# pagmerek/frave

Measured on AMD Instinct MI355X. Metric: Mpixels/s encode (transform+quant) at 4096x4096, higher is better.
Workload: dtype u8->i32

## Files before the change

frave_amd/csrc/fri_hip.cpp:

```cpp
#include "fri_hip_internal.hpp"

#include <atomic>
#include <cstdio>
#include <cstdlib>
#include <mutex>
#include <new>
#include <optional>
#include <thread>

#include "search_scaffold.hpp"
#include "solve6.hpp"

using namespace fri;
using namespace fri::host;

void PlanDelete::operator()(fri_hip_plan *p) const { delete p; }

struct fri_hip_multi {
    std::vector<fri_hip_ctx *> ctxs;
    std::vector<fri_hip_plan *> plans;
};

namespace {

// ... 12 lines not shown
std::vector<float> laplace_table() {
    static const float width[10] = {2.5f, 4.5f, 6.3f, 8.5f, 12.7f, 16.f, 20.f, 24.f, 28.f, 36.f};
    std::vector<float> t(10 * 1024);
    for (int b = 0; b < 10; b++)
        for (uint32_t j = 0; j < 1024; j++) {
            const float x = (float)((j & 1u) ? (int32_t)(j + 1) / -2 : (int32_t)(j / 2));
            t[b * 1024 + j] = std::exp(-std::fabs(x - 0.0f) / width[b]) / (2.0f * width[b]);
        }
    return t;
}

struct Knobs {
    int band_rows = 0, cells_per_tile = 0, cells_per_wg = 0, target_wgs = 0, tile_bytes = 0;
    int ranks = 0;
    std::optional<int> strided_shares;
    bool has_rank_weights = false;
    float rank_weight[4] = {0, 0, 0, 0};
    bool pins_forward = false;
    int batch_share_tiles = 0;
    std::optional<int> inv_shared, inv_strided_shares;
    int inv_band_rows = 0;
    int pred_blocks = 0, hist_blocks = 0, trace = 0, k3_scan = 0;
    int k1_ablate = 0, k2_ablate = 0, k3_ablate = 0, k4_ablate = 0;
    std::optional<int> k1_cached_stores, k1_batch_shares, k4_older_eighths;
};

Knobs read_knobs() {
    Knobs k;
    const char *on = std::getenv("FRI_HIP_TUNING");
    if (!on || on[0] != '1' || on[1] != 0) return k;
    auto env = [](const char *name) { return std::getenv(name); };
    auto pin = [&](const char *name) {
        const char *s = env(name);
        k.pins_forward |= s != nullptr;
        return s;
    };
    auto opt = [](const char *s) { return s ? std::optional<int>(std::atoi(s)) : std::nullopt; };
    auto num = [&](const char *s) { return opt(s).value_or(0); };
    k.band_rows = num(pin("FRI_HIP_BAND_ROWS")), k.cells_per_tile = num(pin("FRI_HIP_CELLS_PER_TILE")), k.cells_per_wg = num(pin("FRI_HIP_CELLS_PER_WG"));
    k.target_wgs = num(pin("FRI_HIP_TARGET_WGS")), k.tile_bytes = num(pin("FRI_HIP_TILE_BYTES")), k.ranks = std::min(num(pin("FRI_HIP_RANKS")), 4);
    k.strided_shares = opt(pin("FRI_HIP_STRIDED_SHARES"));
    if (const char *s = pin("FRI_HIP_RANK_WEIGHTS")) {
        float *w = k.rank_weight;
        k.has_rank_weights = std::sscanf(s, "%f,%f,%f,%f", &w[0], &w[1], &w[2], &w[3]) == 4;
    }
    k.batch_share_tiles = num(env("FRI_HIP_BATCH_SHARE_TILES"));
    k.inv_shared = opt(env("FRI_HIP_INV_SHARED")), k.inv_strided_shares = opt(env("FRI_HIP_INV_STRIDED_SHARES")), k.inv_band_rows = num(env("FRI_HIP_INV_BAND_ROWS"));
    k.pred_blocks = num(env("FRI_HIP_PRED_BLOCKS")), k.hist_blocks = num(env("FRI_HIP_HIST_BLOCKS")), k.trace = num(env("FRI_HIP_TRACE")), k.k3_scan = num(env("FRI_HIP_K3_SCAN"));
    k.k1_ablate = num(env("FRI_HIP_K1_ABLATE")), k.k2_ablate = num(env("FRI_HIP_K2_ABLATE")), k.k3_ablate = num(env("FRI_HIP_K3_ABLATE")), k.k4_ablate = num(env("FRI_HIP_K4_ABLATE"));
    k.k1_cached_stores = opt(env("FRI_HIP_K1_CACHED_STORES")), k.k1_batch_shares = opt(env("FRI_HIP_K1_BATCH_SHARES")), k.k4_older_eighths = opt(env("FRI_HIP_K4_OLDER_EIGHTHS"));
    return k;
}

int acquire_acc(fri_hip_plan *p, hipStream_t stream, uint32_t n_planes = 1) {
    fri_hip_ctx *c = p->ctx;
    HIP_TRY(c, hipSetDevice(c->device));
    if (p->acc_dirty) {
        HIP_TRY(c, hipDeviceSynchronize());
        for (auto &a : p->acc_slots) {
            if (a.pred_acc) HIP_TRY(c, hipMemset(a.pred_acc, 0, (size_t)a.planes * kPredAccWords * sizeof(uint32_t)));
            if (a.fit_acc) HIP_TRY(c, hipMemset(a.fit_acc, 0, (size_t)a.planes * kFitShards * kFitAccWords * sizeof(unsigned long long)));
        }
        HIP_TRY(c, hipDeviceSynchronize());
        p->acc_dirty = false;
    }
    int idx = -1;
    for (uint32_t i = 0; i < kPredAccRing && idx < 0; i++)
        if (p->acc_slots[i].used && p->acc_slots[i].stream == stream) idx = (int)i;
    for (uint32_t i = 0; i < kPredAccRing && idx < 0; i++)
        if (!p->acc_slots[i].used) {
            p->acc_slots[i].used = true;
            p->acc_slots[i].stream = stream;
            idx = (int)i;
// ... 480 lines not shown
            (e = upload(bufs, gi.inv_parts, d.inv_parts, kInvListPad)))
            return fail_hip(ctx, e, "inverse lists");
        d.inv_rect_bytes = gi.inv_rect_bytes;
    }
    d.F = (uint32_t)g.centers.size(), d.width = (int32_t)g.width, d.height = (int32_t)g.height, d.channels = (int32_t)g.channels, d.n_pred_tiles = g.n_pred_tiles;
    d.covers_image = g.n_valid_leaves == (uint64_t)g.width * g.height;
    d.inv_group = fwd.many_shares && g.wg_tiles.size() > 1 && (g.wg_tiles.size() - 1) % 1024 == 0 ? (int32_t)((g.wg_tiles.size() - 1) / 1024) : 1;
    d.inv_max_wg_tiles = d.inv_group > 1 ? 0 : d.max_wg_tiles, d.inv_max_wg_cells = d.inv_group > 1 ? 0 : d.max_wg_cells;
    for (size_t sh = 0; d.inv_group > 1 && sh + d.inv_group < g.wg_tiles.size(); sh += d.inv_group) {
        const Tile &first = g.tiles[g.wg_tiles[sh]], &last = g.tiles[g.wg_tiles[sh + d.inv_group] - 1];
        d.inv_max_wg_cells = std::max(d.inv_max_wg_cells, last.cell_begin + last.cell_count - first.cell_begin);
        d.inv_max_wg_tiles = std::max(d.inv_max_wg_tiles, g.wg_tiles[sh + d.inv_group] - g.wg_tiles[sh]);
    }
    d.pred_blocks = k.pred_blocks > 0 ? (uint32_t)k.pred_blocks : (uint32_t)ctx->cu_count;
    d.hist_blocks = k.hist_blocks > 0 ? (uint32_t)k.hist_blocks : 2u * (uint32_t)ctx->cu_count;
    d.k1_ablate = k.k1_ablate;
    if (k.k1_cached_stores) d.k1_cached_stores = *k.k1_cached_stores > 0 ? 1 : 0;
    if (k.k1_batch_shares) d.k1_batch_shares = *k.k1_batch_shares != 0;
    d.k2_ablate = k.k2_ablate;
    d.k3_ablate = k.k3_ablate;
    d.k3_scan = k.k3_scan > 0;
    d.k4_ablate = k.k4_ablate;
    if (k.k4_older_eighths) d.k4_older_eighths = *k.k4_older_eighths;
    if (hipMalloc(bufs.emplace_back().put(), (size_t)d.pred_blocks * kPredJunkWaves * kPredJunkBytes) != hipSuccess) return FRI_HIP_ERR_HIP;
    d.junk = static_cast<uint8_t *>(bufs.back().get());
    if (k.trace > 0) {
        const size_t bytes = (size_t)std::max<size_t>(d.n_wg, p->own_inverse_tiling ? gi.wg_tiles.size() : 0) * 16 * sizeof(unsigned long long);
        auto &t = bufs.emplace_back();
        if (hipMalloc(t.put(), bytes) != hipSuccess || hipMemset(t, 0, bytes) != hipSuccess) return FRI_HIP_ERR_HIP;
        d.trace = static_cast<unsigned long long *>(t.get());
    }
    if (hipEventCreate(p->ev_begin.put()) != hipSuccess || hipEventCreate(p->ev_end.put()) != hipSuccess) return FRI_HIP_ERR_HIP;
    p->dev_inv = d;
    if (p->own_inverse_tiling && (e = upload_tiling(bufs, gi, p->dev_inv, true))) return fail_hip(ctx, e, "inverse tiling");
    p->fwd_tunable = p->own_inverse_tiling && !fwd.many_shares && !d.trace && !k.pins_forward;
    if (p->fwd_tunable) adopt_cached_forward_tiling(p);
    *out = plan.release();
    return FRI_HIP_OK;
}

int fri_hip_plan_destroy(fri_hip_plan *p) {
    if (p && p->ctx) (void)hipSetDevice(p->ctx->device);
    delete p;
    return FRI_HIP_OK;
}

// ... 543 lines not shown
    const bool direct = d_node_words == nullptr;
    if (direct && !compact) return FRI_HIP_ERR_INVALID_ARGUMENT;
    if (compact) coef_stride = image;
    if (direct) word_stride = image;
    if (n_images > 1 && (pixel_stride < fri_hip_plan_pixel_bytes(p) || coef_stride < image || word_stride < image || symbol_stride < (size_t)C * n)) return FRI_HIP_ERR_INVALID_ARGUMENT;
    if (C > 1 && n_images > 1 && (coef_stride != image || word_stride != image || symbol_stride != (size_t)C * n)) return FRI_HIP_ERR_INVALID_ARGUMENT;
    QMatrix q;
    if (int rc = check_q(qmatrix, q)) return rc;
    hipStream_t s = (hipStream_t)stream;
    if (int rc = refuse_capture(p, s)) return rc;
    HIP_TRY(p->ctx, hipSetDevice(p->ctx->device));
    std::optional<Coefs16Lease> lease;
    if (compact && lease.emplace(p, s, (size_t)n_images * C).rc) return lease->rc;
    HIP_TRY(p->ctx, launch_fwd_transform_quant(p->dev, n_images, d_pixels, pixel_stride, d_coefs, coef_stride, q, s, chain_wants_cached_coefficients(p, n_images, fit),
                                               compact ? p->coefs16.get() : nullptr));
    PredBatch b;
    b.n_planes = n_images * C;
    b.coefs = d_coefs;
    b.coefs16 = compact ? p->coefs16.get() : nullptr;
    b.coef_stride = C > 1 || compact ? plane : coef_stride;
    b.out_stride = C > 1 ? plane : word_stride;
    b.params = reinterpret_cast<const PredictParams *>(d_params);
    b.words = d_node_words;
    if (direct) b.words = d_symbols, b.out_stride = C > 1 ? n : symbol_stride, b.stream_pos = p->d_stream_pos;
    if (fit)
        if (int rc = fit_chain(p, b, (unsigned long long *)d_fit_out_of_range, s, nullptr, nullptr, kPredForwardOutput)) return rc;
    if (int rc = predict_launch(p, b, nullptr, nullptr, d_hist, d_n_out_of_alphabet, kPredForwardOutput, s)) return rc;
    if (!direct) HIP_TRY(p->ctx, launch_symbol_gather(p->d_stream_order, n, b.n_planes, d_node_words, b.out_stride, d_symbols, C > 1 ? n : symbol_stride, s));
    return FRI_HIP_OK;
}

int fri_hip_fit_value_params_batch_dev(fri_hip_plan *p, uint32_t n_planes, const int64_t *d_gram, float *d_params, void *stream) {
    if (int rc = need_device(p)) return rc;
    if (!d_gram || !d_params || !n_planes || n_planes > 65535u) return FRI_HIP_ERR_INVALID_ARGUMENT;
    HIP_TRY(p->ctx, hipSetDevice(p->ctx->device));
    HIP_TRY(p->ctx, launch_fit_solve(0, n_planes, reinterpret_cast<const unsigned long long *>(d_gram), nullptr, nullptr, d_params, (hipStream_t)stream));
    return FRI_HIP_OK;
}

int fri_hip_fit_width_params_batch_dev(fri_hip_plan *p, uint32_t n_planes, const int64_t *d_wtw, const double *d_wtr, float *d_params, void *stream) {
    if (int rc = need_device(p)) return rc;
    if (!d_wtw || !d_wtr || !d_params || !n_planes || n_planes > 65535u) return FRI_HIP_ERR_INVALID_ARGUMENT;
    HIP_TRY(p->ctx, hipSetDevice(p->ctx->device));
    const uint64_t F = p->geo.centers.size();
    const unsigned long long rows[3] = {F * 256, F * 128, F * 128};
    HIP_TRY(p->ctx, launch_fit_solve(1, n_planes, reinterpret_cast<const unsigned long long *>(d_wtw), d_wtr, rows, d_params, (hipStream_t)stream));
    return FRI_HIP_OK;
}

int fri_hip_fit_params_batch_dev(fri_hip_plan *p, uint32_t n_planes, const int32_t *d_coefs, size_t coef_stride, float *d_params, uint64_t *d_fit_out_of_range, void *stream) {
    if (int rc = need_device(p)) return rc;
// ... 557 lines not shown
```

frave_amd/csrc/k2_predict.hip:

```cpp
#include "gather_common.hpp"

#include <algorithm>
#include <vector>

namespace fri {
namespace {

__device__ __forceinline__ uint32_t f32_as_u32(float x) {
    uint32_t r;
    asm("v_cvt_u32_f32 %0, %1" : "=v"(r) : "v"(x));
    return r;
}
__device__ __forceinline__ int f32_as_i32(float x) {
    int r;
    asm("v_cvt_i32_f32 %0, %1" : "=v"(r) : "v"(x));
    return r;
}
__host__ __device__ constexpr uint32_t bucket_of(uint32_t w) {
    return w < 3 ? 0 : w < 5 ? 1 : w < 6 ? 2 : w < 8 ? 3 : w < 12 ? 4 : w < 16 ? 5 : w < 20 ? 6 : w < 25 ? 7 : w < 30 ? 8 : 9;
}
__host__ __device__ constexpr uint32_t bucket_plane(int bit) {
    uint32_t m = 0;
    for (uint32_t w = 0; w < 32; w++) m |= ((bucket_of(w) >> bit) & 1u) << w;
    return m;
// ... 14 lines not shown
    const uint16_t *nbr_table;
    const uint32_t *pred_off;
    const uint16_t *pair_pos;
    const uint16_t *heap_of_pos;
    const uint32_t *halo_list;
    uint32_t *inexact;
    size_t coef_stride, out_stride;
    const PredictParams *params;
    int32_t ablate;
    const uint8_t *interior;
    const uint32_t *valid_mask;
    uint8_t *bucket;
    int32_t *prediction;
    uint32_t *hist;
    unsigned long long *n_oob;
    uint8_t *junk;
    unsigned long long *trace;
    uint32_t *acc;
    int8_t lf_delta[8];
    uint32_t serial;
    uint32_t n_tiles;
    uint16_t *words;
    const uint32_t *stream_pos;
    int32_t trusted;
    PredictParams pp;
    PredictParams pp3[3];
};

constexpr int kAccZeroFlag = 0, kAccTicket = 12, kAccInexact = 14;
constexpr uint32_t kPredZeroBlocks = 10;
static_assert(kAccInexact + 2 == (int)kPredAccWords && kAccZeroFlag + (int)kPredZeroBlocks <= kAccTicket, "accumulator layout");
__device__ __forceinline__ void pred_clear_issue(const PredArgs &a, int tid, int n_threads) {
    const uint32_t nz = min(gridDim.x, kPredZeroBlocks);
    if (blockIdx.x >= nz) return;
    for (uint32_t c = blockIdx.x; c < 10u; c += nz)
        for (uint32_t j = (uint32_t)tid; j < 1024u; j += (uint32_t)n_threads) (void)__hip_atomic_exchange(a.hist + c * 1024u + j, 0u, __ATOMIC_RELAXED, __HIP_MEMORY_SCOPE_AGENT);
    if (blockIdx.x == 0 && tid == 0) (void)__hip_atomic_exchange(a.n_oob, 0ull, __ATOMIC_RELAXED, __HIP_MEMORY_SCOPE_AGENT);
}
__device__ __forceinline__ void pred_clear_publish(const PredArgs &a, int tid) {
    if (blockIdx.x < min(gridDim.x, kPredZeroBlocks) && tid == 0)
        (void)__hip_atomic_exchange(a.acc + kAccZeroFlag + blockIdx.x, a.serial, __ATOMIC_RELAXED, __HIP_MEMORY_SCOPE_AGENT);
}
__device__ __forceinline__ uint32_t pred_clear_poll(const PredArgs &a, int lane) {
    return (uint32_t)lane < min(gridDim.x, kPredZeroBlocks) ? __hip_atomic_load(a.acc + kAccZeroFlag + lane, __ATOMIC_RELAXED, __HIP_MEMORY_SCOPE_AGENT) : a.serial;
}
template <bool CHECK>
// ... 95 lines not shown
    width = __fadd_rn(width, __fmul_rn(q.w[3], fabsf(__fsub_rn(f[4], f[5]))));
    width = __fadd_rn(width, __fmul_rn(q.w[4], fabsf(__fsub_rn(f[1], f[5]))));
    width = __fadd_rn(width, __fmul_rn(q.w[5], fabsf(__fsub_rn(f[2], f[4]))));
    pf = __fmul_rn(f[0], q.v[0]);
    pf = __fadd_rn(pf, __fmul_rn(f[1], q.v[1]));
    pf = __fadd_rn(pf, __fmul_rn(f[2], q.v[2]));
    pf = __fadd_rn(pf, __fmul_rn(f[3], q.v[3]));
    pf = __fadd_rn(pf, __fmul_rn(f[4], q.v[4]));
    pf = __fadd_rn(pf, __fmul_rn(f[5], q.v[5]));
}

__device__ __forceinline__ void p3_lf(int v0, int v1, int v2, uint32_t &b12, int &prediction) {
    const uint32_t w = (uint32_t)iabs_w(sub_w(v0, v2));
    const int mx = max(v0, v2), mn = min(v0, v2);
    prediction = v1 >= mx ? mx : v1 <= mn ? mn : sub_w(add_w(v0, v2), v1);
    b12 = bucket_of_rt(w) << 12;
}

template <int ROLE>
__device__ __forceinline__ int p3_node_of(int lane, int n) {
    return ROLE ? 256 + 4 * lane + n : 128 * (n >> 1) + 2 * lane + (n & 1);
}

template <int IMG, int ROLE, int CELL, bool WORDS, bool STREAM = false>
__device__ __forceinline__ void p3_half(const uint32_t (&addr)[4][6], float (&ga)[6], float (&gb)[6], const int (&own)[4], const PredictParams &pp, bool interior, uint32_t some4,
                                        int lane, uint32_t *s_hist, const uint16_t *s_bkt, uint8_t *bd, int32_t *pd, uint16_t *wd, uint8_t *junk, int ablate,
                                        const uint32_t (&pos)[4] = {0, 0, 0, 0}, bool has = true) {
    constexpr int kOff = IMG * kP3ImageBytes + CELL * kP3SlotBytes;
    uint32_t b12[4], bin[4], sym[4];
    int pred[4];
    const uint32_t bkt_lds = (uint32_t)(uintptr_t)(__attribute__((address_space(3))) const uint16_t *)s_bkt;
    uint32_t tbl_addr[4];
    p3_issue<kOff>(ga, addr[0]);
#pragma unroll
    for (int j = 0; j < 4; j++) {
        float(&g)[6] = (j & 1) ? gb : ga;
        float(&gn)[6] = (j & 1) ? ga : gb;
        if (j == 0) __builtin_amdgcn_s_setprio(CELL ? 1 : 3);
        if (j == 2) __builtin_amdgcn_s_setprio(CELL ? 0 : 2);
        if (j == 0)
            p3_issue_wait<kOff>(gn, addr[1], g);
        else if (j < 3)
            p3_issue_wait_tbl<kOff>(gn, addr[j + 1], g, b12[j - 1], tbl_addr[j - 1]);
        else
            p3_wait_tbl(g, b12[2], tbl_addr[2]);
        if (j > 0) bin[j - 1] = b12[j - 1] + (sym[j - 1] << 2);
        const P3Group q = p3_group(pp, ROLE ? 0 : j < 2 ? 2 : 1);
        float width, pf;
        p3_node_math(g, q, width, pf);
        tbl_addr[j] = bkt_lds + 2u * min(f32_as_u32(width), 31u);
// ... 10 lines not shown
    if (ablate & 4) pred[0] ^= (int)(bin[0] ^ bin[1] ^ bin[2] ^ bin[3]);
    auto leave = [&](const int (&pr)[4], const uint32_t (&bk)[4]) {
        if (WORDS && STREAM) {
            if (!has) return;
#pragma unroll
            for (int j = 0; j < 4; j++) {
                const bool lf = ROLE == 0 && j < 2 && lane == 0;
                const bool some = interior ? !lf : ((some4 >> j) & 1u) != 0;
                if (some && !(ablate & 32)) wd[pos[j]] = (uint16_t)(bin[j] >> 2);
            }
            return;
        }
        if (WORDS) {
            const uint32_t w01 = (bin[1] << 14) | (bin[0] >> 2), w23 = (bin[3] << 14) | (bin[2] >> 2);
            if (ROLE) {
                if (!(ablate & 32) || ((w01 ^ w23) == 0x12345678)) __builtin_nontemporal_store(i32x2{(int)w01, (int)w23}, reinterpret_cast<i32x2 *>(wd + 256) + lane);
            } else {
                uint32_t *q01 = lane == 0 ? reinterpret_cast<uint32_t *>(junk) : reinterpret_cast<uint32_t *>(wd) + lane;
                if (!(ablate & 32) || ((w01 ^ w23) == 0x12345678)) {
                    __builtin_nontemporal_store(w01, q01);
                    __builtin_nontemporal_store(w23, reinterpret_cast<uint32_t *>(wd + 128) + lane);
                }
            }
            return;
        }
        if (ROLE) {
            const uint32_t lo = __builtin_amdgcn_perm(bk[1], bk[0], 0x0C0C0501u), hi = __builtin_amdgcn_perm(bk[3], bk[2], 0x05010C0Cu);
            if (!(ablate & 32) || ((lo ^ hi ^ pr[0] ^ pr[1] ^ pr[2] ^ pr[3]) == 0x12345678)) {
                __builtin_nontemporal_store(i32x4{pr[0], pr[1], pr[2], pr[3]}, reinterpret_cast<i32x4 *>(pd + 256) + lane);
                __builtin_nontemporal_store((lo | hi) >> 4, reinterpret_cast<uint32_t *>(bd + 256) + lane);
            }
        } else {
            const uint32_t lo = __builtin_amdgcn_perm(bk[1], bk[0], 0x0C0C0501u) >> 4, hi = __builtin_amdgcn_perm(bk[3], bk[2], 0x0C0C0501u) >> 4;
            i32x2 *p01 = lane == 0 ? reinterpret_cast<i32x2 *>(junk + 512) : reinterpret_cast<i32x2 *>(pd) + lane;
            uint16_t *b01 = lane == 0 ? reinterpret_cast<uint16_t *>(junk) : reinterpret_cast<uint16_t *>(bd) + lane;
            if (!(ablate & 32) || ((lo ^ hi ^ pr[0] ^ pr[1] ^ pr[2] ^ pr[3]) == 0x12345678)) {
                __builtin_nontemporal_store(i32x2{pr[0], pr[1]}, p01);
                __builtin_nontemporal_store((uint16_t)lo, b01);
                __builtin_nontemporal_store(i32x2{pr[2], pr[3]}, reinterpret_cast<i32x2 *>(pd + 128) + lane);
                __builtin_nontemporal_store((uint16_t)hi, reinterpret_cast<uint16_t *>(bd + 128) + lane);
            }
        }
    };
    if (__builtin_expect(interior, 1)) {
#pragma unroll
        for (int j = 0; j < 4; j++) {
// ... 29 lines not shown
#pragma unroll
    for (int k = 0; k < 3; k++) {
        const int d0 = a.lf_delta[k], d1 = a.lf_delta[3 + k];
        const int delta = it.node ? d1 : d0;
        const int r = row[slot + (delta == kLfNever ? 0 : delta)];
        it.nb[k] = delta == kLfNever ? -1 : r;
    }
    if (!active) it.raw = -1;
}
struct P3LfValues {
    int v[3], value;
    uint32_t mask0;
};
template <bool C16 = false>
__device__ __forceinline__ void p3_lf_hop_b(const PredArgs &a, const int32_t *plane, const P3LfItem &it, P3LfValues &x) {
    const uint32_t n = (uint32_t)it.node;
    auto at = [&](int cell) -> int { return C16 ? (int)(reinterpret_cast<const int16_t *>(plane) + (size_t)cell * kCell)[n] : (plane + (size_t)cell * kCell)[n]; };
#pragma unroll
    for (int k = 0; k < 3; k++) x.v[k] = at(max(pred_slot_cell(it.nb[k]), 0));
    const int cell = max(pred_slot_cell(it.raw), 0);
    x.value = at(cell);
    x.mask0 = a.valid_mask[(size_t)cell * 16];
}
template <bool WORDS, bool STREAM = false>
__device__ __forceinline__ void p3_lf_finish(const PredArgs &a, uint32_t *s_hist, const P3LfItem &it, const P3LfValues &x) {
    const int cell = pred_slot_cell(it.raw);
    if (cell < 0) return;
    int v[3];
#pragma unroll
    for (int k = 0; k < 3; k++) v[k] = it.nb[k] < 0 || x.v[k] == kNone ? 0 : x.v[k];
    uint32_t b12;
    int prediction;
    p3_lf(v[0], v[1], v[2], b12, prediction);
    const bool some = pred_slot_interior(it.raw) || ((x.mask0 >> it.node) & 1u);
    const uint32_t sym = pack_signed(sub_w(x.value, prediction));
    const uint32_t counter = sym < 1024u ? (b12 >> 2) + sym : (uint32_t)kHistBins;
    if (some) atomicAdd(&s_hist[counter], 1u);
    if (WORDS && STREAM) {
        if (some) a.words[a.stream_pos[(size_t)cell * kCell + it.node]] = (uint16_t)counter;
        return;
    }
    if (WORDS) {
        a.words[(size_t)cell * kCell + it.node] = (uint16_t)counter;
        return;
    }
    if (a.prediction) a.prediction[(size_t)cell * kCell + it.node] = some ? prediction : 0;
    if (a.bucket) a.bucket[(size_t)cell * kCell + it.node] = (uint8_t)(some ? b12 >> 12 : 0u);
}

struct ExactArgs {
    const int32_t *coefs;
    const uint16_t *nbr_table;
    const int32_t *nbr_cells;
    const uint8_t *interior;
    const uint32_t *valid_mask;
    uint8_t *bucket;
    int32_t *prediction;
    uint32_t *hist;
    unsigned long long *n_oob;
    uint32_t *acc;
    uint32_t F;
    PredictParams pp;
    size_t coef_stride, out_stride;
    const PredictParams *params;
    PredictParams pp3[3];
};
// ... 142 lines not shown
        if (ROLE) {
            const i32x2 d = reinterpret_cast<const i32x2 *>(cell_base + 256)[lane];
            return i32x4{d.x, d.y, 0, 0};
        }
        return i32x4{reinterpret_cast<const int32_t *>(cell_base)[lane], reinterpret_cast<const int32_t *>(cell_base + 128)[lane], 0, 0};
    }
    const int32_t *cell_base = plane + cell * kCell;
    if (ROLE) return reinterpret_cast<const i32x4 *>(cell_base + 256)[lane];
    const i32x2 a = reinterpret_cast<const i32x2 *>(cell_base)[lane], b = reinterpret_cast<const i32x2 *>(cell_base + 128)[lane];
    return i32x4{a.x, a.y, b.x, b.y};
}
template <bool C16>
__device__ __forceinline__ void p3_unpack_own(i32x4 &v) {
    if (C16) v = i32x4{(int)(short)v.x, v.x >> 16, (int)(short)v.y, v.y >> 16};
}
template <int ROLE>
__device__ __forceinline__ u32x4 p3_load_pos(const uint32_t *stream_pos, size_t cell, uint32_t lane) {
    const uint32_t *base = stream_pos + cell * kCell;
    if (ROLE) return reinterpret_cast<const u32x4 *>(base + 256)[lane];
    const i32x2 a = reinterpret_cast<const i32x2 *>(base)[lane], b = reinterpret_cast<const i32x2 *>(base + 128)[lane];
    return u32x4{(uint32_t)a.x, (uint32_t)a.y, (uint32_t)b.x, (uint32_t)b.y};
}

template <int IMG, int ROLE, bool CHECK, bool WORDS, bool C16 = false, bool STREAM = false>
__device__ __forceinline__ void p3_tile(const PredArgs &a, const int32_t *plane, P3Lds &lds, int it, bool more, uint32_t next2_tile, int tid, int lane, int wave, int slot_a,
                                        const P3Lane &L, float (&ga)[6], float (&gb)[6], const i32x4 (&own_cur)[2], i32x4 (&own_nxt)[2], const u32x4 (&pos_cur)[2],
                                        u32x4 (&pos_nxt)[2]) {
    uint32_t *s_hist = lds.hist;
    const uint16_t *s_bkt = lds.bkt;
    const int32_t *cur_slots = lds.ring[it % 3], *nxt_slots = lds.ring[(it + 1) % 3];
    const int32_t slot_pre = a.pred_slots[(size_t)next2_tile * kPredSlots + tid % kPredSlots];
    uint32_t st_own_mask[2];
    P3Halo st_halo;
    int raw_own[2] = {-1, -1};
    if (ablate_flags(a.ablate) & 2) more = false;
    if (more) {
#pragma unroll
        for (int c = 0; c < 2; c++) {
            raw_own[c] = __builtin_amdgcn_readfirstlane(nxt_slots[slot_a + c]);
            const int cell = max(pred_slot_cell(raw_own[c]), 0);
            own_nxt[c] = p3_load_own<ROLE, C16>(plane, (size_t)cell, (uint32_t)lane);
            if (STREAM) pos_nxt[c] = p3_load_pos<ROLE>(a.stream_pos, (size_t)cell, (uint32_t)lane);
            if (ROLE == 1) st_own_mask[c] = (a.valid_mask + (size_t)cell * 16)[(uint32_t)lane & 15u];
        }
        p3_issue_halo<C16>(plane, nxt_slots, L.halo_ring, L.halo_heap, st_halo);
    }

#pragma unroll
    for (int c = 0; c < 2; c++) {
        const int raw = (ablate_flags(a.ablate) & 1) ? -1 : __builtin_amdgcn_readfirstlane(cur_slots[slot_a + c]);
        const int cell = pred_slot_cell(raw);
        const bool has = cell >= 0, interior = pred_slot_interior(raw);
        const size_t junk = ((size_t)blockIdx.x * kP3Waves + wave) * kPredJunkBytes;
        uint8_t *bd = has && a.bucket ? a.bucket + (size_t)cell * kCell : a.junk + junk;
        int32_t *pd = has && a.prediction ? a.prediction + (size_t)cell * kCell : reinterpret_cast<int32_t *>(a.junk + junk + 512);
        uint16_t *wd = WORDS && STREAM ? a.words : WORDS && has ? a.words + (size_t)cell * kCell : reinterpret_cast<uint16_t *>(a.junk + junk + 512);
        const uint32_t pos4[4] = {pos_cur[c].x, pos_cur[c].y, pos_cur[c].z, pos_cur[c].w};
        uint32_t some4 = 0;
        if (!interior && has) {
            const uint32_t *m = lds.masks[IMG][slot_a + c];
            if (ROLE) {
                some4 = (m[8 + (lane >> 3)] >> (4 * (lane & 7))) & 15u;
            } else {
                some4 = ((m[lane >> 4] >> (2 * (lane & 15))) & 3u) | (((m[4 + (lane >> 4)] >> (2 * (lane & 15))) & 3u) << 2);
                if (lane == 0) some4 &= ~3u;
            }
        }
        const int own4[4] = {own_cur[c].x, own_cur[c].y, own_cur[c].z, own_cur[c].w};
        if (WORDS && (ablate_flags(a.ablate) & 1)) {
            if (ROLE) {
                __builtin_nontemporal_store(i32x2{0, 0}, reinterpret_cast<i32x2 *>(wd + 256) + lane);
            } else {
                __builtin_nontemporal_store(0u, reinterpret_cast<uint32_t *>(wd) + lane);
                __builtin_nontemporal_store(0u, reinterpret_cast<uint32_t *>(wd + 128) + lane);
            }
        } else if (ablate_flags(a.ablate) & 1) {
            if (ROLE) {
                __builtin_nontemporal_store(i32x4{0, 0, 0, 0}, reinterpret_cast<i32x4 *>(pd + 256) + lane);
                __builtin_nontemporal_store(0u, reinterpret_cast<uint32_t *>(bd + 256) + lane);
            } else {
                __builtin_nontemporal_store(i32x2{0, 0}, reinterpret_cast<i32x2 *>(pd) + lane);
                __builtin_nontemporal_store((uint16_t)0, reinterpret_cast<uint16_t *>(bd) + lane);
                __builtin_nontemporal_store(i32x2{0, 0}, reinterpret_cast<i32x2 *>(pd + 128) + lane);
                __builtin_nontemporal_store((uint16_t)0, reinterpret_cast<uint16_t *>(bd + 128) + lane);
            }
        } else if (c == 0) {
            p3_half<IMG, ROLE, 0, WORDS, STREAM>(L.addr, ga, gb, own4, a.pp, interior, some4, lane, s_hist, s_bkt, bd, pd, wd, a.junk + junk, ablate_flags(a.ablate), pos4, has);
        } else {
            p3_half<IMG, ROLE, 1, WORDS, STREAM>(L.addr, ga, gb, own4, a.pp, interior, some4, lane, s_hist, s_bkt, bd, pd, wd, a.junk + junk, ablate_flags(a.ablate), pos4, has);
        }
    }

    if (more) {
        asm volatile("" : "+v"(own_nxt[0]), "+v"(own_nxt[1]), "+v"(st_halo.v));
        if (STREAM) asm volatile("" : "+v"(pos_nxt[0]), "+v"(pos_nxt[1]));
        p3_unpack_own<C16>(own_nxt[0]), p3_unpack_own<C16>(own_nxt[1]);
        uint32_t nxt_img = IMG ^ 1;
        asm volatile("" : "+s"(nxt_img));
        uint8_t *nxt = lds.cells[0] + nxt_img * kP3ImageBytes;
        uint32_t *nxt_masks = &lds.masks[0][0][0] + nxt_img * (kPredSlots * 16);
        float m = 0.f;
#pragma unroll
        for (int c = 0; c < 2; c++) {
            m = __builtin_fmaxf(m, p3_commit4<CHECK>(raw_own[c], own_nxt[c], nxt + (slot_a + c) * kP3SlotBytes, L.opos[0], L.opos[1]));
            if (ROLE == 1 && lane < 16) nxt_masks[(slot_a + c) * 16 + lane] = st_own_mask[c];
        }
        m = __builtin_fmaxf(m, p3_commit_halo<CHECK>(st_halo, nxt, L.halo_lds));
        if (CHECK) p3_check(m, lane, a.inexact);
    }
    if (tid < kPredSlots) lds.ring[(it + 2) % 3][tid] = slot_pre;
    lds_barrier();
    trace_stamp(a.trace, blockIdx.x, 2 + it, tid);
}

template <int ROLE, bool CHECK, bool WORDS, bool C16 = false, bool STREAM = false>
__device__ __forceinline__ void p3_run(const PredArgs &a, P3Lds &lds, int tid, int lane, int wave, uint32_t &early_poll) {
    uint8_t *s_cells = lds.cells[0];
    int32_t *s_ring = &lds.ring[0][0];
    uint32_t *s_masks = &lds.masks[0][0][0];
    const int pair = wave >> 1;
    const int slot_a = (1 + (pair >> 1)) * kPredSide + 1 + 2 * (pair & 1);
    const int32_t *plane = a.coefs;

    P3Lane L;
    const uint32_t cells_lds = (uint32_t)(uintptr_t)(__attribute__((address_space(3))) uint8_t *)s_cells;
#pragma unroll
    for (int j = 0; j < 4; j++) {
        const u32x4 o = reinterpret_cast<const u32x4 *>(a.pred_off)[p3_node_of<ROLE>(lane, j)];
        const uint32_t rel[3] = {o.x, o.y, o.z};
#pragma unroll
        for (int k = 0; k < 6; k++) {
            const int r = (int)(short)((rel[k >> 1] >> (16 * (k & 1))) & 0xFFFFu);
            L.addr[j][k] = r == 0x7FFF ? cells_lds + kP3ZeroOff : cells_lds + (uint32_t)(slot_a * kP3SlotBytes + r);
        }
    }
    L.opos[0] = 4u * a.pair_pos[ROLE ? 128 + 2 * lane : lane];
    L.opos[1] = 4u * a.pair_pos[ROLE ? 129 + 2 * lane : 64 + lane];
    {
// ... 10 lines not shown
        pred_clear_publish(a, tid);
        return;
    }
    const uint32_t last = walk.first + ((walk.end - 1 - walk.first) / walk.step) * walk.step;
    constexpr uint32_t kLfTilesPerPass = kP3Threads / 2 / 32;
    const uint32_t my_tiles = (walk.end - walk.first + walk.step - 1u) / walk.step;
    const int lf_tid = (wave >> 1) * 64 + lane;
    P3LfItem lf_item;
    if (ROLE == 1) p3_lf_hop_a(a, walk.first + (uint32_t)(lf_tid >> 5) * walk.step, (uint32_t)(lf_tid >> 5) < my_tiles, lf_tid, lf_item);
    if (tid < kPredSlots) {
        s_ring[tid] = a.pred_slots[(size_t)walk.first * kPredSlots + tid];
        s_ring[kPredSlots + tid] = a.pred_slots[(size_t)min(walk.first + walk.step, last) * kPredSlots + tid];
    }
    wait_for_own_memory_ops_then_barrier();
    pred_clear_publish(a, tid);
    {
        uint32_t st_own_mask[2] = {0, 0};
        int raw_own[2];
#pragma unroll
        for (int c = 0; c < 2; c++) {
            raw_own[c] = __builtin_amdgcn_readfirstlane(s_ring[slot_a + c]);
            const int cell = max(pred_slot_cell(raw_own[c]), 0);
            own_a[c] = p3_load_own<ROLE, C16>(plane, (size_t)cell, (uint32_t)lane);
            if (STREAM) pos_a[c] = p3_load_pos<ROLE>(a.stream_pos, (size_t)cell, (uint32_t)lane);
            if (ROLE == 1) st_own_mask[c] = (a.valid_mask + (size_t)cell * 16)[(uint32_t)lane & 15u];
        }
        P3Halo st_halo;
        p3_issue_halo<C16>(plane, s_ring, L.halo_ring, L.halo_heap, st_halo);
        P3LfValues lf_values;
        if (ROLE == 1) p3_lf_hop_b<C16>(a, plane, lf_item, lf_values);
        p3_unpack_own<C16>(own_a[0]), p3_unpack_own<C16>(own_a[1]);
        float m = 0.f;
#pragma unroll
        for (int c = 0; c < 2; c++) {
            m = __builtin_fmaxf(m, p3_commit4<CHECK>(raw_own[c], own_a[c], s_cells + (slot_a + c) * kP3SlotBytes, L.opos[0], L.opos[1]));
            if (ROLE == 1 && lane < 16) s_masks[(slot_a + c) * 16 + lane] = st_own_mask[c];
        }
        m = __builtin_fmaxf(m, p3_commit_halo<CHECK>(st_halo, s_cells, L.halo_lds));
        if (CHECK) p3_check(m, lane, a.inexact);
        if (ROLE == 1 && !(ablate_flags(a.ablate) & 1)) p3_lf_finish<WORDS, STREAM>(a, lds.hist, lf_item, lf_values);
    }
    if (ROLE == 1) {
        for (uint32_t base = kLfTilesPerPass; base < my_tiles; base += kLfTilesPerPass) {
            const uint32_t k = base + (uint32_t)(lf_tid >> 5);
            P3LfItem it;
            P3LfValues x;
            p3_lf_hop_a(a, walk.first + k * walk.step, k < my_tiles, lf_tid, it);
            p3_lf_hop_b<C16>(a, plane, it, x);
            if (!(ablate_flags(a.ablate) & 1)) p3_lf_finish<WORDS, STREAM>(a, lds.hist, it, x);
        }
    }
    lds_barrier();
    trace_stamp(a.trace, blockIdx.x, 1, tid);
    early_poll = pred_clear_poll(a, lane);

    int it = 0;
    for (uint32_t tile = walk.first; tile < walk.end;) {
        p3_tile<0, ROLE, CHECK, WORDS, C16, STREAM>(a, plane, lds, it, tile + walk.step < walk.end, min(tile + 2 * walk.step, last), tid, lane, wave, slot_a, L, ga, gb, own_a, own_b, pos_a, pos_b);
        tile += walk.step, it++;
        if (tile >= walk.end) break;
        p3_tile<1, ROLE, CHECK, WORDS, C16, STREAM>(a, plane, lds, it, tile + walk.step < walk.end, min(tile + 2 * walk.step, last), tid, lane, wave, slot_a, L, ga, gb, own_b, own_a, pos_b, pos_a);
        tile += walk.step, it++;
    }
}

__device__ __forceinline__ PredArgs pred_plane_view(const PredArgs &a0, uint32_t plane) {
    PredArgs a = a0;
    a.coefs += plane * a0.coef_stride;
    if (a.bucket) a.bucket += plane * a0.out_stride;
    if (a.prediction) a.prediction += plane * a0.out_stride;
    if (a.words) a.words += plane * a0.out_stride;
    a.hist += (size_t)plane * kHistBins;
    a.n_oob += plane;
    a.acc += (size_t)plane * kPredAccWords;
    a.inexact = a.acc + kAccInexact;
    if (a0.params)
        a.pp = a0.params[plane];
    else if (plane == 0)
        a.pp = a0.pp3[0];
    else if (plane == 1)
        a.pp = a0.pp3[1];
    else
        a.pp = a0.pp3[2];
    return a;
}

template <bool CHECK, bool WORDS, bool C16 = false, bool STREAM = false>
__global__ void __launch_bounds__(kP3Threads) predict_histogram_kernel3(const PredArgs a0) {
    PredArgs a = pred_plane_view(a0, blockIdx.y);
    if (C16) a.coefs = reinterpret_cast<const int32_t *>(reinterpret_cast<const int16_t *>(a0.coefs) + blockIdx.y * a0.coef_stride);
    __shared__ __attribute__((aligned(16))) P3Lds lds;
    uint32_t *s_hist = lds.hist;
    uint8_t *s_cells = lds.cells[0];
    int32_t *s_ring = &lds.ring[0][0];
    uint16_t *s_bkt = lds.bkt;
    const int tid = threadIdx.x, lane = tid & 63;
    const int wave = __builtin_amdgcn_readfirstlane(tid >> 6);
    trace_stamp(a.trace, blockIdx.x, 0, tid);
    pred_clear_issue(a, tid, kP3Threads);
    for (int i = tid; i < kHistBins + 4; i += kP3Threads) s_hist[i] = 0;
    if (tid < 32) s_bkt[tid] = (uint16_t)(bucket_of((uint32_t)tid) << 12);
    for (int i = tid; i < 2 * (kP3ImageBytes - kP3ZeroOff) / 4; i += kP3Threads)
        reinterpret_cast<uint32_t *>(s_cells + (i / ((kP3ImageBytes - kP3ZeroOff) / 4)) * kP3ImageBytes + kP3ZeroOff)[i % ((kP3ImageBytes - kP3ZeroOff) / 4)] = 0;
    uint32_t early_poll = 0;
    if (wave & 1)
        p3_run<1, CHECK, WORDS, C16, STREAM>(a, lds, tid, lane, wave, early_poll);
    else
        p3_run<0, CHECK, WORDS, C16, STREAM>(a, lds, tid, lane, wave, early_poll);
    lds_barrier();
    trace_stamp(a.trace, blockIdx.x, 13, tid);
    pred_hand_over<CHECK>(a, s_hist, reinterpret_cast<uint32_t *>(s_ring), tid, kP3Threads, early_poll);
    trace_exit(a.trace, blockIdx.x, tid);
}

}


void build_lf_deltas(const uint16_t *nbr_table, int8_t *out ) {
    for (int node = 0; node < 2; node++)
        for (int k = 0; k < 3; k++) {
            const uint32_t e = nbr_table[node * 6 + k];
            const int s7 = (e >> 9) & 7;
            const int da = (int)((0x0F14u >> (2 * s7)) & 3u), db = (int)((0x14F0u >> (2 * s7)) & 3u);
            out[node * 3 + k] = (e & 0x8000u) ? (int8_t)kLfNever : (int8_t)(((da & 1) - (da & 2)) * kPredSide + ((db & 1) - (db & 2)));
        }
    out[6] = out[7] = 0;
}

void build_gather_tables(const uint16_t *nbr_table, uint32_t *gather_off , uint16_t *pair_pos , uint16_t *heap_of_pos ) {
    static const uint16_t kPairPos[256] = {
#include "gather_layout.inc"
// ... 67 lines not shown
    a.hist = hist;
    a.n_oob = n_oob;
    a.n_tiles = p.n_pred_tiles;
    a.trusted = trust != kPredAnyInt32 ? 1 : 0;
    a.words = b.words;
    if (b.words && trust != kPredForwardOutput) return hipErrorInvalidValue;
    uint32_t blocks = p.n_pred_tiles < p.pred_blocks ? p.n_pred_tiles : p.pred_blocks;
    if (b.n_planes > 1) {
        const uint32_t share = (p.n_pred_tiles + 7) / 8, eighth = p.pred_blocks / 8 ? p.pred_blocks / 8 : 1;
        blocks = share < eighth ? eighth : share;
        if (blocks > p.pred_blocks) blocks = p.pred_blocks;
        if (blocks > p.n_pred_tiles) blocks = p.n_pred_tiles;
    }
    if (!blocks) blocks = 1;
    a.junk = p.junk;
    a.trace = p.trace;
    a.pred_off = p.gather_off;
    a.pair_pos = p.pair_pos;
    a.heap_of_pos = p.heap_of_pos;
    a.halo_list = p.halo_list;
    a.ablate = p.k2_ablate;
    (void)hipGetLastError();
    a.stream_pos = b.stream_pos;
    if (b.stream_pos && !(b.words && b.coefs16)) return hipErrorInvalidValue;
    if (b.words && b.coefs16 && b.stream_pos)
        hipLaunchKernelGGL((predict_histogram_kernel3<false, true, true, true>), dim3(blocks, b.n_planes), dim3(kP3Threads), 0, stream, a);
    else if (b.words && b.coefs16)
        hipLaunchKernelGGL((predict_histogram_kernel3<false, true, true>), dim3(blocks, b.n_planes), dim3(kP3Threads), 0, stream, a);
    else if (b.words)
        hipLaunchKernelGGL((predict_histogram_kernel3<false, true>), dim3(blocks, b.n_planes), dim3(kP3Threads), 0, stream, a);
    else if (trust == kPredForwardOutput)
        hipLaunchKernelGGL((predict_histogram_kernel3<false, false>), dim3(blocks, b.n_planes), dim3(kP3Threads), 0, stream, a);
    else
        hipLaunchKernelGGL((predict_histogram_kernel3<true, false>), dim3(blocks, b.n_planes), dim3(kP3Threads), 0, stream, a);
    e = hipGetLastError();
    if (e != hipSuccess || trust != kPredAnyInt32) return e;
    ExactArgs x{};
    x.coefs = b.coefs;
    x.coef_stride = b.coef_stride;
    x.out_stride = b.out_stride;
    x.params = b.params;
    for (int k = 0; k < 3; k++) x.pp3[k] = b.pp[k];
    x.nbr_table = p.nbr_table;
    x.nbr_cells = p.nbr_cells;
    x.interior = p.interior;
    x.valid_mask = p.valid_mask;
    x.bucket = bucket;
    x.prediction = prediction;
// ... 12 lines not shown
```

frave_amd/csrc/kernels.hpp:

```cpp
#pragma once
#include <hip/hip_runtime_api.h>

#include <cstddef>
#include <cstdint>

#include "geometry.hpp"

namespace fri {

struct DevicePlan {
    const Tile *tiles = nullptr;
    const int32_t *tile_cells = nullptr;
    const TileCell *tile_meta = nullptr;
    const int32_t *wg_tiles = nullptr;
    const int32_t *wg_tiles_batch = nullptr;
    uint32_t n_wg_batch = 0;
    uint32_t n_wg = 0;
    int32_t max_tile_cells = 0;
    bool covers_image = false;
    int32_t max_wg_tiles = 0;
    int32_t max_wg_cells = 0;
    int32_t inv_group = 1;
    int32_t inv_max_wg_tiles = 0, inv_max_wg_cells = 0;
    const Int2 *centers = nullptr;
// ... 15 lines not shown
    uint32_t pred_blocks = 0;
    uint32_t n_tiles = 0;
    uint32_t F = 0;
    int32_t width = 0, height = 0, channels = 0;
    int32_t lds_pitch = 0, lds_rows = 0, cells_per_tile = 0;
    bool k1_batch_shares = true;
    int k1_cached_stores = -1;
    int32_t k1_ablate = 0;
    int32_t k2_ablate = 0;
    bool rct = false;
    bool ycc = false;
    bool k3_multiply = false;
    bool k3_midpoint = false;
    unsigned long long *trace = nullptr;
    bool k1_measuring = false;
    unsigned long long *k1_xcd_stat = nullptr;
    const InvTileLists *inv_lists = nullptr;
    const uint16_t *inv_quads = nullptr, *inv_dwords = nullptr;
    const uint32_t *inv_parts = nullptr;
    int32_t inv_rect_bytes = 0;
    bool k3_scan = false;
    int32_t k3_ablate = 0;
    int32_t k4_ablate = 0;
    int32_t k4_older_eighths = 5;
};

constexpr uint32_t kPredJunkWaves = 16, kPredJunkBytes = 2560;
constexpr uint32_t kFitAccWords = 3 * 28 + 18 + 2;
constexpr uint32_t kFitShards = 16;
constexpr uint32_t kPredAccRing = 8, kPredAccWords = 16;

struct QMatrix {
    int32_t q[32];
};

struct PredictParams {
    float value[3][6];
    float width[3][6];
};

hipError_t launch_fwd_transform_quant(const DevicePlan &p, uint32_t n_images, const uint8_t *pixels, size_t pixel_stride, int32_t *coefs,
                                      size_t coef_stride, const QMatrix &q, hipStream_t stream, bool cached_stores = false,
                                      int16_t *coefs16 = nullptr );
struct PredBatch {
    uint32_t n_planes = 1;
    const int32_t *coefs = nullptr;
    const int16_t *coefs16 = nullptr;
    size_t coef_stride = 0, out_stride = 0;
    const PredictParams *params = nullptr;
    PredictParams pp[3] = {};
    const uint32_t *stream_pos = nullptr;
    uint16_t *words = nullptr;
};
constexpr int kPredAnyInt32 = 0, kPredPromised = 1, kPredForwardOutput = 2;
hipError_t launch_predict_histogram(const DevicePlan &p, uint32_t *acc, uint32_t serial, const PredBatch &b, uint8_t *bucket, int32_t *prediction, uint32_t *hist,
                                    unsigned long long *n_oob, int trust, hipStream_t stream);
struct FitSolve {
    float *params = nullptr;
    float *host_params = nullptr;
    unsigned long long *host_range = nullptr;
    unsigned long long rows[3] = {0, 0, 0};
};
hipError_t launch_fit_accumulate(const DevicePlan &p, unsigned long long *acc, int mode, const PredBatch &b, unsigned long long *sums_int, double *sums_dbl,
                                 unsigned long long *out_of_range, hipStream_t stream, const FitSolve *solve = nullptr, int trust = 0 );
hipError_t launch_fit_solve(int mode, uint32_t n_planes, const unsigned long long *sums_int, const double *sums_dbl, const unsigned long long rows[3], float *params,
                            hipStream_t stream, float *host_params = nullptr, const unsigned long long *range = nullptr, unsigned long long *host_range = nullptr);
hipError_t launch_inverse_transform(const DevicePlan &p, uint32_t n_images, const int32_t *coefs, size_t coef_stride, const QMatrix &q, uint8_t *pixels, size_t pixel_stride,
                                    hipStream_t stream, unsigned long long *measure = nullptr);

hipError_t launch_symbol_gather(const uint32_t *order, uint64_t n_symbols, uint32_t n_planes, const uint16_t *words, size_t word_stride, uint16_t *out, size_t stream_stride,
                                hipStream_t stream);
hipError_t launch_symbol_stream(const uint32_t *order, uint64_t n_symbols, uint32_t n_planes, const int32_t *coefs, size_t coef_stride, const uint8_t *bucket,
                                const int32_t *prediction, size_t out_stride, uint16_t *out, size_t stream_stride, hipStream_t stream);

// ... 56 lines not shown
```

Measured before the change: 919,200.

## Scatter symbols into stream order inside predict kernel when working set is small

When the non-direct, non-compact encode path has a scan footprint below a configurable threshold (default 128 MiB), the predict kernel writes each symbol both to the node-ordered words buffer and directly to its stream position, and the separate symbol-gather kernel launch is skipped. This removes one kernel launch and a full read/write pass over the symbol buffer, at the cost of extra scattered halfword stores and stream-position loads inside the predict kernel. Larger workloads keep the old gather pass.

```diff
diff --git a/frave_amd/csrc/fri_hip.cpp b/frave_amd/csrc/fri_hip.cpp
--- a/frave_amd/csrc/fri_hip.cpp
+++ b/frave_amd/csrc/fri_hip.cpp
@@ -58,7 +58,7 @@
     int inv_band_rows = 0;
     int pred_blocks = 0, hist_blocks = 0, trace = 0, k3_scan = 0;
     int k1_ablate = 0, k2_ablate = 0, k3_ablate = 0, k4_ablate = 0;
-    std::optional<int> k1_cached_stores, k1_batch_shares, k4_older_eighths;
+    std::optional<int> k1_cached_stores, k1_batch_shares, k4_older_eighths, symbols_gather_mib;
 };
 
 Knobs read_knobs() {
@@ -85,6 +85,7 @@
     k.pred_blocks = num(env("FRI_HIP_PRED_BLOCKS")), k.hist_blocks = num(env("FRI_HIP_HIST_BLOCKS")), k.trace = num(env("FRI_HIP_TRACE")), k.k3_scan = num(env("FRI_HIP_K3_SCAN"));
     k.k1_ablate = num(env("FRI_HIP_K1_ABLATE")), k.k2_ablate = num(env("FRI_HIP_K2_ABLATE")), k.k3_ablate = num(env("FRI_HIP_K3_ABLATE")), k.k4_ablate = num(env("FRI_HIP_K4_ABLATE"));
     k.k1_cached_stores = opt(env("FRI_HIP_K1_CACHED_STORES")), k.k1_batch_shares = opt(env("FRI_HIP_K1_BATCH_SHARES")), k.k4_older_eighths = opt(env("FRI_HIP_K4_OLDER_EIGHTHS"));
+    k.symbols_gather_mib = opt(env("FRI_HIP_SYMBOLS_GATHER_MIB"));
     return k;
 }
 
@@ -611,6 +612,7 @@
     d.k3_scan = k.k3_scan > 0;
     d.k4_ablate = k.k4_ablate;
     if (k.k4_older_eighths) d.k4_older_eighths = *k.k4_older_eighths;
+    if (k.symbols_gather_mib) d.symbols_gather_mib = std::max(*k.symbols_gather_mib, 0);
     if (hipMalloc(bufs.emplace_back().put(), (size_t)d.pred_blocks * kPredJunkWaves * kPredJunkBytes) != hipSuccess) return FRI_HIP_ERR_HIP;
     d.junk = static_cast<uint8_t *>(bufs.back().get());
     if (k.trace > 0) {
@@ -1200,11 +1202,16 @@
     b.out_stride = C > 1 ? plane : word_stride;
     b.params = reinterpret_cast<const PredictParams *>(d_params);
     b.words = d_node_words;
-    if (direct) b.words = d_symbols, b.out_stride = C > 1 ? n : symbol_stride, b.stream_pos = p->d_stream_pos;
+    const size_t scan_bytes = ((size_t)b.n_planes * (4 + 2 + 2) + 4) * plane;
+    const bool gather = !direct && !compact && scan_bytes > ((size_t)p->dev.symbols_gather_mib << 20);
+    if (direct)
+        b.words = d_symbols, b.out_stride = C > 1 ? n : symbol_stride, b.stream_pos = p->d_stream_pos;
+    else if (!gather)
+        b.stream = d_symbols, b.stream_stride = C > 1 ? n : symbol_stride, b.stream_pos = p->d_stream_pos;
     if (fit)
         if (int rc = fit_chain(p, b, (unsigned long long *)d_fit_out_of_range, s, nullptr, nullptr, kPredForwardOutput)) return rc;
     if (int rc = predict_launch(p, b, nullptr, nullptr, d_hist, d_n_out_of_alphabet, kPredForwardOutput, s)) return rc;
-    if (!direct) HIP_TRY(p->ctx, launch_symbol_gather(p->d_stream_order, n, b.n_planes, d_node_words, b.out_stride, d_symbols, C > 1 ? n : symbol_stride, s));
+    if (gather) HIP_TRY(p->ctx, launch_symbol_gather(p->d_stream_order, n, b.n_planes, d_node_words, b.out_stride, d_symbols, C > 1 ? n : symbol_stride, s));
     return FRI_HIP_OK;
 }
 
diff --git a/frave_amd/csrc/k2_predict.hip b/frave_amd/csrc/k2_predict.hip
--- a/frave_amd/csrc/k2_predict.hip
+++ b/frave_amd/csrc/k2_predict.hip
@@ -60,6 +60,8 @@
     uint32_t n_tiles;
     uint16_t *words;
     const uint32_t *stream_pos;
+    uint16_t *stream;
+    size_t stream_stride;
     int32_t trusted;
     PredictParams pp;
     PredictParams pp3[3];
@@ -201,10 +203,11 @@
     return ROLE ? 256 + 4 * lane + n : 128 * (n >> 1) + 2 * lane + (n & 1);
 }
 
-template <int IMG, int ROLE, int CELL, bool WORDS, bool STREAM = false>
+template <int IMG, int ROLE, int CELL, bool WORDS, bool STREAM = false, bool BOTH = false>
 __device__ __forceinline__ void p3_half(const uint32_t (&addr)[4][6], float (&ga)[6], float (&gb)[6], const int (&own)[4], const PredictParams &pp, bool interior, uint32_t some4,
                                         int lane, uint32_t *s_hist, const uint16_t *s_bkt, uint8_t *bd, int32_t *pd, uint16_t *wd, uint8_t *junk, int ablate,
-                                        const uint32_t (&pos)[4] = {0, 0, 0, 0}, bool has = true) {
+                                        const uint32_t (&pos)[4] = {0, 0, 0, 0}, bool has = true, uint16_t *sd = nullptr) {
+    static_assert(!BOTH || (WORDS && !STREAM), "BOTH: the halfword form next to the stream, not the stream form itself");
     constexpr int kOff = IMG * kP3ImageBytes + CELL * kP3SlotBytes;
     uint32_t b12[4], bin[4], sym[4];
     int pred[4];
@@ -261,6 +264,15 @@
                     __builtin_nontemporal_store(w23, reinterpret_cast<uint32_t *>(wd + 128) + lane);
                 }
             }
+            if (BOTH) {
+#pragma unroll
+                for (int j = 0; j < 4; j++) {
+                    const bool lf = ROLE == 0 && j < 2 && lane == 0;
+                    const bool some = interior ? !lf : has ? ((some4 >> j) & 1u) != 0 : true;
+                    const uint32_t at = has ? pos[j] : 4u * (uint32_t)lane + (uint32_t)j;
+                    if (some && !(ablate & 32)) sd[at] = (uint16_t)(bin[j] >> 2);
+                }
+            }
             return;
         }
         if (ROLE) {
@@ -336,7 +348,7 @@
     x.value = at(cell);
     x.mask0 = a.valid_mask[(size_t)cell * 16];
 }
-template <bool WORDS, bool STREAM = false>
+template <bool WORDS, bool STREAM = false, bool BOTH = false>
 __device__ __forceinline__ void p3_lf_finish(const PredArgs &a, uint32_t *s_hist, const P3LfItem &it, const P3LfValues &x) {
     const int cell = pred_slot_cell(it.raw);
     if (cell < 0) return;
@@ -356,6 +368,7 @@
     }
     if (WORDS) {
         a.words[(size_t)cell * kCell + it.node] = (uint16_t)counter;
+        if (BOTH && some) a.stream[a.stream_pos[(size_t)cell * kCell + it.node]] = (uint16_t)counter;
         return;
     }
     if (a.prediction) a.prediction[(size_t)cell * kCell + it.node] = some ? prediction : 0;
@@ -544,7 +557,7 @@
     return u32x4{(uint32_t)a.x, (uint32_t)a.y, (uint32_t)b.x, (uint32_t)b.y};
 }
 
-template <int IMG, int ROLE, bool CHECK, bool WORDS, bool C16 = false, bool STREAM = false>
+template <int IMG, int ROLE, bool CHECK, bool WORDS, bool C16 = false, bool STREAM = false, bool BOTH = false>
 __device__ __forceinline__ void p3_tile(const PredArgs &a, const int32_t *plane, P3Lds &lds, int it, bool more, uint32_t next2_tile, int tid, int lane, int wave, int slot_a,
                                         const P3Lane &L, float (&ga)[6], float (&gb)[6], const i32x4 (&own_cur)[2], i32x4 (&own_nxt)[2], const u32x4 (&pos_cur)[2],
                                         u32x4 (&pos_nxt)[2]) {
@@ -562,7 +575,7 @@
             raw_own[c] = __builtin_amdgcn_readfirstlane(nxt_slots[slot_a + c]);
             const int cell = max(pred_slot_cell(raw_own[c]), 0);
             own_nxt[c] = p3_load_own<ROLE, C16>(plane, (size_t)cell, (uint32_t)lane);
-            if (STREAM) pos_nxt[c] = p3_load_pos<ROLE>(a.stream_pos, (size_t)cell, (uint32_t)lane);
+            if (STREAM || BOTH) pos_nxt[c] = p3_load_pos<ROLE>(a.stream_pos, (size_t)cell, (uint32_t)lane);
             if (ROLE == 1) st_own_mask[c] = (a.valid_mask + (size_t)cell * 16)[(uint32_t)lane & 15u];
         }
         p3_issue_halo<C16>(plane, nxt_slots, L.halo_ring, L.halo_heap, st_halo);
@@ -577,6 +590,7 @@
         uint8_t *bd = has && a.bucket ? a.bucket + (size_t)cell * kCell : a.junk + junk;
         int32_t *pd = has && a.prediction ? a.prediction + (size_t)cell * kCell : reinterpret_cast<int32_t *>(a.junk + junk + 512);
         uint16_t *wd = WORDS && STREAM ? a.words : WORDS && has ? a.words + (size_t)cell * kCell : reinterpret_cast<uint16_t *>(a.junk + junk + 512);
+        uint16_t *sd = !BOTH ? nullptr : has ? a.stream : reinterpret_cast<uint16_t *>(a.junk + junk + 1536);
         const uint32_t pos4[4] = {pos_cur[c].x, pos_cur[c].y, pos_cur[c].z, pos_cur[c].w};
         uint32_t some4 = 0;
         if (!interior && has) {
@@ -607,15 +621,15 @@
                 __builtin_nontemporal_store((uint16_t)0, reinterpret_cast<uint16_t *>(bd + 128) + lane);
             }
         } else if (c == 0) {
-            p3_half<IMG, ROLE, 0, WORDS, STREAM>(L.addr, ga, gb, own4, a.pp, interior, some4, lane, s_hist, s_bkt, bd, pd, wd, a.junk + junk, ablate_flags(a.ablate), pos4, has);
+            p3_half<IMG, ROLE, 0, WORDS, STREAM, BOTH>(L.addr, ga, gb, own4, a.pp, interior, some4, lane, s_hist, s_bkt, bd, pd, wd, a.junk + junk, ablate_flags(a.ablate), pos4, has, sd);
         } else {
-            p3_half<IMG, ROLE, 1, WORDS, STREAM>(L.addr, ga, gb, own4, a.pp, interior, some4, lane, s_hist, s_bkt, bd, pd, wd, a.junk + junk, ablate_flags(a.ablate), pos4, has);
+            p3_half<IMG, ROLE, 1, WORDS, STREAM, BOTH>(L.addr, ga, gb, own4, a.pp, interior, some4, lane, s_hist, s_bkt, bd, pd, wd, a.junk + junk, ablate_flags(a.ablate), pos4, has, sd);
         }
     }
 
     if (more) {
         asm volatile("" : "+v"(own_nxt[0]), "+v"(own_nxt[1]), "+v"(st_halo.v));
-        if (STREAM) asm volatile("" : "+v"(pos_nxt[0]), "+v"(pos_nxt[1]));
+        if (STREAM || BOTH) asm volatile("" : "+v"(pos_nxt[0]), "+v"(pos_nxt[1]));
         p3_unpack_own<C16>(own_nxt[0]), p3_unpack_own<C16>(own_nxt[1]);
         uint32_t nxt_img = IMG ^ 1;
         asm volatile("" : "+s"(nxt_img));
@@ -635,7 +649,7 @@
     trace_stamp(a.trace, blockIdx.x, 2 + it, tid);
 }
 
-template <int ROLE, bool CHECK, bool WORDS, bool C16 = false, bool STREAM = false>
+template <int ROLE, bool CHECK, bool WORDS, bool C16 = false, bool STREAM = false, bool BOTH = false>
 __device__ __forceinline__ void p3_run(const PredArgs &a, P3Lds &lds, int tid, int lane, int wave, uint32_t &early_poll) {
     uint8_t *s_cells = lds.cells[0];
     int32_t *s_ring = &lds.ring[0][0];
@@ -692,7 +706,7 @@
             raw_own[c] = __builtin_amdgcn_readfirstlane(s_ring[slot_a + c]);
             const int cell = max(pred_slot_cell(raw_own[c]), 0);
             own_a[c] = p3_load_own<ROLE, C16>(plane, (size_t)cell, (uint32_t)lane);
-            if (STREAM) pos_a[c] = p3_load_pos<ROLE>(a.stream_pos, (size_t)cell, (uint32_t)lane);
+            if (STREAM || BOTH) pos_a[c] = p3_load_pos<ROLE>(a.stream_pos, (size_t)cell, (uint32_t)lane);
             if (ROLE == 1) st_own_mask[c] = (a.valid_mask + (size_t)cell * 16)[(uint32_t)lane & 15u];
         }
         P3Halo st_halo;
@@ -708,7 +722,7 @@
         }
         m = __builtin_fmaxf(m, p3_commit_halo<CHECK>(st_halo, s_cells, L.halo_lds));
         if (CHECK) p3_check(m, lane, a.inexact);
-        if (ROLE == 1 && !(ablate_flags(a.ablate) & 1)) p3_lf_finish<WORDS, STREAM>(a, lds.hist, lf_item, lf_values);
+        if (ROLE == 1 && !(ablate_flags(a.ablate) & 1)) p3_lf_finish<WORDS, STREAM, BOTH>(a, lds.hist, lf_item, lf_values);
     }
     if (ROLE == 1) {
         for (uint32_t base = kLfTilesPerPass; base < my_tiles; base += kLfTilesPerPass) {
@@ -717,7 +731,7 @@
             P3LfValues x;
             p3_lf_hop_a(a, walk.first + k * walk.step, k < my_tiles, lf_tid, it);
             p3_lf_hop_b<C16>(a, plane, it, x);
-            if (!(ablate_flags(a.ablate) & 1)) p3_lf_finish<WORDS, STREAM>(a, lds.hist, it, x);
+            if (!(ablate_flags(a.ablate) & 1)) p3_lf_finish<WORDS, STREAM, BOTH>(a, lds.hist, it, x);
         }
     }
     lds_barrier();
@@ -726,10 +740,10 @@
 
     int it = 0;
     for (uint32_t tile = walk.first; tile < walk.end;) {
-        p3_tile<0, ROLE, CHECK, WORDS, C16, STREAM>(a, plane, lds, it, tile + walk.step < walk.end, min(tile + 2 * walk.step, last), tid, lane, wave, slot_a, L, ga, gb, own_a, own_b, pos_a, pos_b);
+        p3_tile<0, ROLE, CHECK, WORDS, C16, STREAM, BOTH>(a, plane, lds, it, tile + walk.step < walk.end, min(tile + 2 * walk.step, last), tid, lane, wave, slot_a, L, ga, gb, own_a, own_b, pos_a, pos_b);
         tile += walk.step, it++;
         if (tile >= walk.end) break;
-        p3_tile<1, ROLE, CHECK, WORDS, C16, STREAM>(a, plane, lds, it, tile + walk.step < walk.end, min(tile + 2 * walk.step, last), tid, lane, wave, slot_a, L, ga, gb, own_b, own_a, pos_b, pos_a);
+        p3_tile<1, ROLE, CHECK, WORDS, C16, STREAM, BOTH>(a, plane, lds, it, tile + walk.step < walk.end, min(tile + 2 * walk.step, last), tid, lane, wave, slot_a, L, ga, gb, own_b, own_a, pos_b, pos_a);
         tile += walk.step, it++;
     }
 }
@@ -740,6 +754,7 @@
     if (a.bucket) a.bucket += plane * a0.out_stride;
     if (a.prediction) a.prediction += plane * a0.out_stride;
     if (a.words) a.words += plane * a0.out_stride;
+    if (a.stream) a.stream += plane * a0.stream_stride;
     a.hist += (size_t)plane * kHistBins;
     a.n_oob += plane;
     a.acc += (size_t)plane * kPredAccWords;
@@ -755,7 +770,7 @@
     return a;
 }
 
-template <bool CHECK, bool WORDS, bool C16 = false, bool STREAM = false>
+template <bool CHECK, bool WORDS, bool C16 = false, bool STREAM = false, bool BOTH = false>
 __global__ void __launch_bounds__(kP3Threads) predict_histogram_kernel3(const PredArgs a0) {
     PredArgs a = pred_plane_view(a0, blockIdx.y);
     if (C16) a.coefs = reinterpret_cast<const int32_t *>(reinterpret_cast<const int16_t *>(a0.coefs) + blockIdx.y * a0.coef_stride);
@@ -774,9 +789,9 @@
         reinterpret_cast<uint32_t *>(s_cells + (i / ((kP3ImageBytes - kP3ZeroOff) / 4)) * kP3ImageBytes + kP3ZeroOff)[i % ((kP3ImageBytes - kP3ZeroOff) / 4)] = 0;
     uint32_t early_poll = 0;
     if (wave & 1)
-        p3_run<1, CHECK, WORDS, C16, STREAM>(a, lds, tid, lane, wave, early_poll);
+        p3_run<1, CHECK, WORDS, C16, STREAM, BOTH>(a, lds, tid, lane, wave, early_poll);
     else
-        p3_run<0, CHECK, WORDS, C16, STREAM>(a, lds, tid, lane, wave, early_poll);
+        p3_run<0, CHECK, WORDS, C16, STREAM, BOTH>(a, lds, tid, lane, wave, early_poll);
     lds_barrier();
     trace_stamp(a.trace, blockIdx.x, 13, tid);
     pred_hand_over<CHECK>(a, s_hist, reinterpret_cast<uint32_t *>(s_ring), tid, kP3Threads, early_poll);
@@ -890,8 +905,14 @@
     a.ablate = p.k2_ablate;
     (void)hipGetLastError();
     a.stream_pos = b.stream_pos;
-    if (b.stream_pos && !(b.words && b.coefs16)) return hipErrorInvalidValue;
-    if (b.words && b.coefs16 && b.stream_pos)
+    a.stream = b.stream;
+    a.stream_stride = b.stream_stride;
+    if ((b.stream_pos && !(b.words && (b.coefs16 || b.stream))) || (b.stream && !(b.words && b.stream_pos))) return hipErrorInvalidValue;
+    if (b.words && b.stream && b.coefs16)
+        hipLaunchKernelGGL((predict_histogram_kernel3<false, true, true, false, true>), dim3(blocks, b.n_planes), dim3(kP3Threads), 0, stream, a);
+    else if (b.words && b.stream)
+        hipLaunchKernelGGL((predict_histogram_kernel3<false, true, false, false, true>), dim3(blocks, b.n_planes), dim3(kP3Threads), 0, stream, a);
+    else if (b.words && b.coefs16 && b.stream_pos)
         hipLaunchKernelGGL((predict_histogram_kernel3<false, true, true, true>), dim3(blocks, b.n_planes), dim3(kP3Threads), 0, stream, a);
     else if (b.words && b.coefs16)
         hipLaunchKernelGGL((predict_histogram_kernel3<false, true, true>), dim3(blocks, b.n_planes), dim3(kP3Threads), 0, stream, a);
diff --git a/frave_amd/csrc/kernels.hpp b/frave_amd/csrc/kernels.hpp
--- a/frave_amd/csrc/kernels.hpp
+++ b/frave_amd/csrc/kernels.hpp
@@ -61,6 +61,7 @@
     bool k3_scan = false;
     int32_t k3_ablate = 0;
     int32_t k4_ablate = 0;
+    int32_t symbols_gather_mib = 128;
     int32_t k4_older_eighths = 5;
 };
 
@@ -89,6 +90,8 @@
     const PredictParams *params = nullptr;
     PredictParams pp[3] = {};
     const uint32_t *stream_pos = nullptr;
+    uint16_t *stream = nullptr;
+    size_t stream_stride = 0;
     uint16_t *words = nullptr;
 };
 constexpr int kPredAnyInt32 = 0, kPredPromised = 1, kPredForwardOutput = 2;
```

Measured after the change: 907,200. 0.987x the previous value.
